# zhouxinlzu/PebbleSDR

Hardware: AMD Instinct MI355X
Metric: IQ Msamples/s through full ProcessBlock chain (higher is better)
Workload: dtype f32; 1 GPU; configs[1]: 20 Msps int8-shape IQ (values k/128, resident in HBM as float2), 1 channel/GPU, mixer+decimate(D=64)+WFM mono demod + 8192-bin SignalSpectrum per 2048-sample frame; frames_per_buffer=2048, spectrum_bins=8192, parallelism=independent channel per GPU, no collectives

## Files before the change

pebblesdr_amd/csrc/cores.hip:

```cpp
#include <cmath>
#include <cstdarg>
#include <cstddef>
#include <hip/hip_ext.h>
#include "kernels_demod.h"
#include "kernels_fastfir.h"
#include "kernels_frontend.h"
#include <algorithm>
#include "kernels_fused_dec.h"
#include "kernels_bank_dec.h"
#include "kernels_spectrum.h"
#include "receiver.h"

namespace pg {

std::string &last_error()
{
    static thread_local std::string e;
    return e;
}
int fail(int code, const char *fmt, ...)
{
    char buf[512];
    va_list ap;
    va_start(ap, fmt);
// ... 699 lines not shown
            }
            bank_state_valid = false;
        }
    }
    const long long len0 = max_in / s0.stride;
    if (ns == 1) {
        if (int rc = buf0.alloc((int)C, last_hist, len0)) return rc;
    } else {
        if (halo0 > 256 * 32) return fail(PEBBLEGPU_E_UNSUPPORTED, "cascade look-back %lld too deep", halo0);
        if (wide) {
            if (!fused_front) { if (int rc = buf0.alloc((int)C, wide_taps - 1, len0)) return rc; }
            if (int rc = buf1.alloc((int)C, (int)halo0, len0 / wide_stride)) return rc;
            if (int rc = fin.alloc((int)C, last_hist, len0 / wide_stride / later)) return rc;
        } else {
            if (int rc = buf0.alloc((int)C, (int)halo0, len0)) return rc;
            if (int rc = fin.alloc((int)C, last_hist, len0 / later)) return rc;
        }
    }
    for (int i = 0; i < 2; i++) {
        PG_HIP(hipMalloc((void **)&d_hist_mixed[i], sizeof(float2) * kMaxTaps * C));
        PG_HIP(hipMemset(d_hist_mixed[i], 0, sizeof(float2) * kMaxTaps * C));
        if (C == 1) {
            PG_HIP(hipMalloc((void **)&d_xtail_w[i], sizeof(float2) * 2048));
            PG_HIP(hipMemset(d_xtail_w[i], 0, sizeof(float2) * 2048));
        }

    }
    return 0;
}
void DecimCore::release()
{
    delete fused_p;
    fused_p = nullptr;
    for (int i = 0; i < 2; i++) {
        if (d_xhist[i]) (void)hipFree(d_xhist[i]);
        d_xhist[i] = nullptr;
    }
    for (int i = 0; i < 2; i++) {
        if (d_y0stage2[i]) (void)hipFree(d_y0stage2[i]);
        d_y0stage2[i] = nullptr;
    }
    d_y0stage = nullptr;
    for (int i = 0; i < 2; i++) {
        if (d_bank_state[i]) (void)hipFree(d_bank_state[i]);
        d_bank_state[i] = nullptr;
    }
    for (int i = 0; i < 2; i++) {
        if (d_dyn[i]) (void)hipFree(d_dyn[i]);
        d_dyn[i] = nullptr;
    }
    buf0.release();
    buf1.release();
    fin.release();
    fin2.release();
    fin3.release();
    if (d_wide_taps) (void)hipFree(d_wide_taps);
    d_wide_taps = nullptr;
    for (int i = 0; i < 2; i++) {
        if (d_hist_mixed[i]) (void)hipFree(d_hist_mixed[i]);
        d_hist_mixed[i] = nullptr;
        if (d_xtail_w[i]) (void)hipFree(d_xtail_w[i]);
        d_xtail_w[i] = nullptr;
    }
    if (d_c0tab) (void)hipFree(d_c0tab);
    d_c0tab = nullptr;
    if (d_ph_scratch) (void)hipFree(d_ph_scratch);
// ... 78 lines not shown
                                                            RawSrc raw)
{
    const int i = blockIdx.x * 256 + threadIdx.x;
    const long long src = n - 2048 + i;
    const float2 v = raw.base ? raw_load(raw, src) : in[src];
    out[i] = cscale(v, window[i]);
}
int DecimCore::run_beside_spectrum(hipStream_t s, const float2 *d_in, long long in_pitch, bool shared_input, long long n, const OscBank &osc, const RawSrc *raw)
{
    const int R = 8;
    const long long j_first = (10 + first.stride - 1) / first.stride;
    const RawSrc rs = raw ? *raw : RawSrc{nullptr, 0, 0, 0.f, 0};
    launch(raw ? k_mix_hb11_bank<false, false, true> : k_mix_hb11_bank<false, false, false>, dim3(len0 / (4LL * R * 64) != 0 ? 2 : 1, 1), dim3(256), s, d_in, in_pitch,
           (int)shared_input, buf0.data(), buf0.pitch, len0, (const ChanOsc *)osc.d_osc, (const float2 *)d_hist_mixed[hist_parity], d_hist_mixed[hist_parity ^ 1],
           (int)kMaxTaps, (const float *)osc.d_amp, osc.a_inf, bank_taps, first.gain, osc.inline_dyn, 0, (int)C, R, j_first, rs);
    PG_HIP(hipGetLastError());
    hist_parity ^= 1;
    xtail_parity ^= 1;
    last_fused = false;
    front_name = "k_spectrum_t128 (decimator inside)";
    rest_name = "";
    return 0;
}
int DecimCore::run(hipStream_t s, const float2 *d_in, long long in_pitch, bool shared_input, long long n, const OscBank &osc,
                   hipEvent_t after_first, const RawSrc *raw, const OscAdvance *oa)
{
    if (raw && !raw_ready(osc)) return fail(PEBBLEGPU_E_INVALID, "raw-format input reached a decimator path that has no converting loads");
    if (n <= 0 || n % (long long)chain.total != 0)
        return fail(PEBBLEGPU_E_SIZE, "%lld samples is not a multiple of the decimation %u", n, chain.total);
    len0 = n / first.stride;
    if (fin3.base && rotate3) { std::swap(fin, fin2); std::swap(fin2, fin3); }
    else if (fin2.base) std::swap(fin, fin2);
    const HistBuf *src = &buf0;
    last_fused = false;
    last_mfma = false;
    osc_advanced = false;
    done_recorded = false;
    const bool had_bank_state = bank_state_valid;
    bank_state_valid = false;
    const bool had_dyn = dyn_valid;
    dyn_valid = false;
    if ((fused_all || bank_mfma) && shared_input && !osc.any_transient()) {
        const HistBuf &y0b = fused_front ? buf1 : buf0;
        if (n / ((long long)first.stride * (fused_front ? wide_stride : 1)) > y0b.cap) return fail(PEBBLEGPU_E_SIZE, "%lld samples exceed this object's capacity", n);
        len_out = n / (long long)chain.total;
        const long long groups = cdiv(C, 64);
        if (bank_mfma && (unsigned long long)n * 8 < 0xFFF00000ull && (unsigned long long)C * (unsigned long long)fin.pitch * 8 < 0xFFF00000ull &&
            len_out >= 64 && (reinterpret_cast<uintptr_t>(d_in) & 7) == 0) {
            dyn_valid = had_dyn;
            if (int rc = run_bank_mfma(s, d_in, n, osc, had_bank_state, oa)) return rc;
            if (after_first) PG_HIP(hipEventRecord(after_first, s));
            return 0;
        }
      if (int rc = flush_y0(s)) return rc;
      if (fused_all) {
        long long L = tun.fused_l > 0 ? tun.fused_l : ((len_out * groups / 704 + 15) & ~15LL);
        if (L < 32) L = 32;
        fused_p->n_out = len_out;
        fused_p->out_pitch = fin.pitch;
        fused_p->y0_pitch = buf0.pitch;
        fused_p->L = (int)L;
        fused_p->a_inf = osc.a_inf;
        launch(k_mix_dec_fused<15, 19, 31>, dim3(cdiv(len_out, L), (unsigned)groups), dim3(256), s, d_in, fin.data(), (const ChanOsc *)osc.d_osc, osc.inline_dyn,
               (const float2 *)d_xhist[hist_parity], d_xhist[hist_parity ^ 1], (const float2 *)buf0.data(), d_y0stage, d_hist_mixed[hist_parity ^ 1], *fused_p);
        PG_HIP(hipGetLastError());
        hist_parity ^= 1;
// ... 5 lines not shown
      }
    }
    if (int rc = flush_y0(s)) return rc;
    if (fused_front) {
        len1 = len0 / wide_stride;
        if (len1 > buf1.cap) return fail(PEBBLEGPU_E_SIZE, "%lld samples exceed this object's capacity", n);
        int cl_log2 = 0;
        while ((1u << cl_log2) < C && cl_log2 < 6) cl_log2++;
        const int R = cl_log2 == 6 ? 16 : 8;
        const dim3 grid(cdiv(len1 + 1, 4LL * R * (64 >> cl_log2)), cdiv(C, 1u << cl_log2));
        const bool uni = cl_log2 == 6 && shared_input;
        auto kern = osc.any_transient() ? (uni ? k_mix_cic_hb<true, true> : k_mix_cic_hb<true, false>) : (uni ? k_mix_cic_hb<false, true> : k_mix_cic_hb<false, false>);
        launch_lds(kern, grid, dim3(256), cl_log2 ? 4 * (size_t)front_tile_slots(cl_log2, R) * sizeof(float2) : 0, s, d_in, in_pitch, (int)shared_input, buf1.data(), buf1.pitch,
                   len1, (const ChanOsc *)osc.d_osc, (const float2 *)d_hist_mixed[hist_parity], d_hist_mixed[hist_parity ^ 1], (int)kMaxTaps,
                   (const float *)osc.d_amp, osc.a_inf, wide_fir, first.stride, 1.0f, osc.inline_dyn, cl_log2, (int)C, R);
        hist_parity ^= 1;
        front_name = "k_mix_cic_hb";
        if (after_first) PG_HIP(hipEventRecord(after_first, s));
        len_out = len1;
        src = &buf1;
    } else {
        if (len0 > buf0.cap) return fail(PEBBLEGPU_E_SIZE, "%lld samples exceed this object's capacity", n);
        if (bank_front && C == 1 && want_lds_free && !osc.any_transient()) {
            const int R = 8;
            const long long j_first = (10 + first.stride - 1) / first.stride;
            const RawSrc rs = raw ? *raw : RawSrc{nullptr, 0, 0, 0.f, 0};
            auto lean = !raw ? k_mix_hb11_lean<-1> : rs.fmt == 0 ? k_mix_hb11_lean<0> : rs.fmt == 1 ? k_mix_hb11_lean<1> : rs.fmt == 2 ? k_mix_hb11_lean<2>
                             : rs.fmt == 3 ? k_mix_hb11_lean<3> : k_mix_hb11_lean<4>;
            const bool edge_launch = tun.lean_edge_launch;
            launch(lean, dim3(cdiv(len0, 4LL * R * 64) + (edge_launch ? 0 : 1)), dim3(256), s, d_in, buf0.data(), len0, (const ChanOsc *)osc.d_osc,
                   osc.a_inf, bank_taps, first.gain, osc.inline_dyn, R, edge_launch ? -j_first : j_first, rs, (const float2 *)d_hist_mixed[hist_parity],
                   d_hist_mixed[hist_parity ^ 1]);
            front_name = "k_mix_hb11_lean";
            if (edge_launch)
                launch(raw ? k_mix_hb11_bank<false, false, true> : k_mix_hb11_bank<false, false, false>, dim3(len0 / (4LL * R * 64) != 0 ? 2 : 1, 1), dim3(256), s, d_in, in_pitch,
                       (int)shared_input, buf0.data(), buf0.pitch, len0, (const ChanOsc *)osc.d_osc, (const float2 *)d_hist_mixed[hist_parity], d_hist_mixed[hist_parity ^ 1],
                       (int)kMaxTaps, (const float *)osc.d_amp, osc.a_inf, bank_taps, first.gain, osc.inline_dyn, 0, (int)C, R, j_first, rs);
        } else if (bank_front && (C >= 16 ? shared_input : want_lds_free)) {
            int cl_log2 = 0;
            while ((1u << cl_log2) < C && cl_log2 < 6) cl_log2++;
            const int R = cl_log2 == 6 ? 16 : 8;
            const dim3 grid(cdiv(len0 + 1, 4LL * R * (64 >> cl_log2)), cdiv(C, 1u << cl_log2));
            const bool uni = cl_log2 == 6;
            auto kern = osc.any_transient() ? (uni ? k_mix_hb11_bank<true, true> : k_mix_hb11_bank<true, false>)
                                            : (uni ? k_mix_hb11_bank<false, true> : k_mix_hb11_bank<false, false>);
            launch_lds(kern, grid, dim3(256), cl_log2 ? 4 * (size_t)front_tile_slots(cl_log2, R) * sizeof(float2) : 0, s, d_in, in_pitch, (int)shared_input, buf0.data(),
                       buf0.pitch, len0, (const ChanOsc *)osc.d_osc, (const float2 *)d_hist_mixed[hist_parity], d_hist_mixed[hist_parity ^ 1], (int)kMaxTaps,
                       (const float *)osc.d_amp, osc.a_inf, bank_taps, first.gain, osc.inline_dyn, cl_log2, (int)C, R, -1LL, RawSrc{nullptr, 0, 0, 0.f, 0});
            front_name = "k_mix_hb11_bank";
        } else {
        const int cg = (first.cic3 && first.stride > 2 && shared_input) ? 8 : 1;
        size_t lds = mixdec_lds_bytes(first);
        if (cg > 1 && lds < (size_t)cg * 258 * sizeof(float4)) lds = (size_t)cg * 258 * sizeof(float4);
        launch_lds(k_mix_dec1, dim3(cdiv(len0, 256), cdiv(C, cg)), dim3(256), lds, s, d_in, in_pitch, (int)shared_input, buf0.data(),
                   buf0.pitch, len0, (const ChanOsc *)osc.d_osc, (const float2 *)d_hist_mixed[hist_parity], (int)kMaxTaps, (const float *)osc.d_amp,
                   osc.a_inf, first, d_hist_mixed[hist_parity ^ 1], osc.inline_dyn, cg, (int)C);
        front_name = "k_mix_dec1";
        }
        hist_parity ^= 1;
        if (after_first) PG_HIP(hipEventRecord(after_first, s));
        len_out = len0;
        if (wide) {
            len1 = len0 / wide_stride;
            launch(k_fir_dec, dim3(cdiv(len1, 256), C), dim3(256), s, (const float2 *)buf0.data(), buf0.pitch, buf1.data(), buf1.pitch, len1, wide_stride,
                   (const float *)d_wide_taps, (const float *)nullptr, 0, (const int *)nullptr, wide_taps, 1.0f, 0, (const int *)nullptr, Gate{nullptr, 0, 0});
            src = &buf1;
        }
    }
    rest_name = wide && !fused_front ? "k_fir_dec" : "";
    if (casc.nst > 0) {
        rest_name = wide && !fused_front ? "k_fir_dec + k_cascade" : "k_cascade";
        len_out = n / (long long)chain.total;
        const bool three2 = casc.nst == 3 && casc.stride[0] == 2 && casc.stride[1] == 2 && casc.stride[2] == 2;
        auto kern = k_cascade<0, 0, 0>;
        if (three2 && casc.ntaps[0] == 15 && casc.ntaps[1] == 23 && casc.ntaps[2] == 47) kern = k_cascade<15, 23, 47>;
        else if (three2 && casc.ntaps[0] == 15 && casc.ntaps[1] == 19 && casc.ntaps[2] == 31) kern = k_cascade<15, 19, 31>;
        launch_lds(kern, dim3(cdiv(len_out, casc.outb), C), dim3(256), casc_lds_bytes, s, (const float2 *)src->data(), src->pitch, fin.data(),
                   fin.pitch, len_out, casc);
    }
    PG_HIP(hipGetLastError());
    if ((fused_all || bank_mfma) && shared_input && n >= xh_depth)
        PG_HIP(hipMemcpyAsync(d_xhist[hist_parity], d_in + (n - xh_depth), sizeof(float2) * xh_depth, hipMemcpyDeviceToDevice, s));
    if (fuse_window && n >= 2048 && shape_for_spectrum()) {
        launch(k_window_tail, dim3(8), dim3(256), s, d_in, n, fuse_window, d_xtail_w[xtail_parity ^ 1], raw ? *raw : RawSrc{nullptr, 0, 0, 0.f, 0});
        xtail_parity ^= 1;
    }
    return 0;
}
void DecimCore::tail_jobs_dec(std::vector<TailJob> &jobs) const
{
    if (last_fused) {
        const HistBuf &y0b = fused_front ? buf1 : buf0;
        if (!last_mfma) jobs.push_back(TailJob{d_y0stage, (long long)fused_hy, (long long)fused_hy, fused_hy, 0, y0b.base + (y0b.hist - fused_hy), y0b.pitch});
        return;
    }
    if (!fused_front && buf0.hist > 0 && casc.nst > 0) jobs.push_back(TailJob{buf0.data(), buf0.pitch, len0, buf0.hist, 0, nullptr, 0});
    if (wide && buf1.hist > 0) jobs.push_back(TailJob{buf1.data(), buf1.pitch, len1, buf1.hist, 0, nullptr, 0});
}
void DecimCore::tail_job_out(std::vector<TailJob> &jobs) const
{
    if (casc.nst == 0) {
        if (!fused_front && buf0.hist > 0) jobs.push_back(TailJob{buf0.data(), buf0.pitch, len0, buf0.hist, 0, nullptr, 0});
        return;
    }
    if (fin.hist <= 0) return;
    if (fin2.base) jobs.push_back(TailJob{fin.data(), fin.pitch, len_out, fin.hist, 0, fin2.base, fin2.pitch});
    else jobs.push_back(TailJob{fin.data(), fin.pitch, len_out, fin.hist, 0, nullptr, 0});
}
void DecimCore::tail_jobs(std::vector<TailJob> &jobs) const
// ... 315 lines not shown
        if (lp_on) ok = design::cascade_impulse(std::vector<double>(), nullptr, std::vector<design::Biquad>(1, l), 1e-11, kWfmLpMax, hl);
        if (ok) ok = design::cascade_impulse(h, &da, std::vector<design::Biquad>(1, br), 1e-11, kWfmIrMax, ha);
        fused = ok && wfm_fir_lds_bytes((int)((ha.size() + 15) & ~(size_t)15), (int)hl.size()) <= 64 * 1024;
        if (fused) {
            L4 = (int)((ha.size() + 15) & ~(size_t)15);
            Llp = (int)hl.size();
            ha.resize((size_t)L4 + 16, 0.0);
            std::vector<float> hlf(hl.begin(), hl.end()), haf(ha.begin(), ha.end());
            PG_HIP(hipMalloc((void **)&d_h, sizeof(float) * (L4 + 16)));
            PG_HIP(hipMemcpy(d_h, haf.data(), sizeof(float) * (L4 + 16), hipMemcpyHostToDevice));
            PG_HIP(hipMalloc((void **)&d_hlp, sizeof(float) * Llp));
            PG_HIP(hipMemcpy(d_hlp, hlf.data(), sizeof(float) * Llp, hipMemcpyHostToDevice));
            for (int i = 0; i < 2; i++) {
                PG_HIP(hipMalloc((void **)&d_xtail[i], sizeof(float2) * (size_t)(L4 + Llp) * C));
                PG_HIP(hipMemset(d_xtail[i], 0, sizeof(float2) * (size_t)(L4 + Llp) * C));
            }
            return 0;
        }
    }
    if (int rc = a.alloc((int)C, 2, max_n)) return rc;
    if (int rc = b.alloc((int)C, kMaxTaps, max_n)) return rc;
    if (int rc = c.alloc((int)C, 0, max_n)) return rc;
    for (int i = 0; i < 2; i++) {
        PG_HIP(hipMalloc((void **)&d_lp_state[i], sizeof(double) * 4 * C));
        PG_HIP(hipMemset(d_lp_state[i], 0, sizeof(double) * 4 * C));
        PG_HIP(hipMalloc((void **)&d_dn_state[i], sizeof(double) * 8 * C));
        PG_HIP(hipMemset(d_dn_state[i], 0, sizeof(double) * 8 * C));
    }
    return 0;
}
void WfmCore::release()
{
    a.release(); b.release(); c.release();
    void *p[] = {d_taps, d_lp_state[0], d_lp_state[1], d_dn_state[0], d_dn_state[1], d_h, d_hlp, d_xtail[0], d_xtail[1], d_stereo, d_pilot, d_hilb, d_stereo_list};
    d_stereo = nullptr;
    d_pilot = nullptr;
    d_hilb = nullptr;
    d_stereo_list = nullptr;
    lm.release();
    rds.release();
    for (void *q : p) if (q) (void)hipFree(q);
    d_taps = nullptr;
    d_lp_state[0] = d_lp_state[1] = d_dn_state[0] = d_dn_state[1] = nullptr;
    d_h = nullptr; d_hlp = nullptr; d_xtail[0] = d_xtail[1] = nullptr;
}
int WfmCore::set_stereo(uint32_t ch, bool on)
{
    if (ch >= C) return fail(PEBBLEGPU_E_INVALID, "channel %u out of range", ch);
    if (on && !fused) return fail(PEBBLEGPU_E_UNSUPPORTED, "dmFMS needs the single-kernel WFM path (this demodulator rate runs the sequential one)");
    if (on && !d_pilot) {
        const design::WfmPilotDesign pd = design::wfm_pilot_design(rate);
        memset(&pilot, 0, sizeof(pilot));
        pilot.b0 = pd.bp.b0; pilot.b2 = pd.bp.b2; pilot.a1 = pd.bp.a1; pilot.a2 = pd.bp.a2;
        pilot.nco_lo = pd.nco_lo; pilot.nco_hi = pd.nco_hi; pilot.alpha = pd.alpha; pilot.beta = pd.beta;
        pilot.err_alpha = pd.err_alpha; pilot.phase_adjust = pd.phase_adjust;
        pilot.L4 = L4;
        PG_HIP(hipMalloc((void **)&d_hilb, sizeof(double) * 122));
        PG_HIP(hipMemcpy(d_hilb, pd.hilb, sizeof(double) * 122, hipMemcpyHostToDevice));
        PG_HIP(hipMalloc((void **)&d_pilot, sizeof(WfmPilotState) * C));
        PG_HIP(hipMalloc((void **)&d_stereo_list, sizeof(int) * C));
        if (int rc = lm.alloc((int)C, L4 + 16, max_n_)) return rc;
        std::vector<WfmPilotState> z(C);
        memset(z.data(), 0, sizeof(WfmPilotState) * C);
        for (auto &q : z) { q.nco_freq = pd.nco_freq0; q.quiet = 1LL << 40; }
        PG_HIP(hipMemcpy(d_pilot, z.data(), sizeof(WfmPilotState) * C, hipMemcpyHostToDevice));
        if (tun.rds) { if (int rc = rds.init(C, rate, max_n_)) return rc; }
    }
// ... 20 lines not shown
int WfmCore::run(hipStream_t s, const float2 *in, long long in_pitch, float2 *out, long long out_pitch, long long n,
                 const std::vector<TailJob> *more_tails, const OscAdvance *oa, bool *carried)
{
    if (carried) *carried = false;
    if (n < kMaxTaps) return fail(PEBBLEGPU_E_SIZE, "WFM demod needs at least %d samples per call", kMaxTaps);
    last_n = n;
    if (stereo_dirty) {
        if (!d_stereo) PG_HIP(hipMalloc((void **)&d_stereo, C));
        PG_HIP(hipMemcpyAsync(d_stereo, stereo.data(), C, hipMemcpyHostToDevice, s));
        std::vector<int> list;
        for (uint32_t ch = 0; ch < C; ch++) if (stereo[ch]) list.push_back((int)ch);
        n_stereo = (int)list.size();
        if (n_stereo) PG_HIP(hipMemcpyAsync(d_stereo_list, list.data(), sizeof(int) * list.size(), hipMemcpyHostToDevice, s));
        PG_HIP(hipStreamSynchronize(s));
        stereo_dirty = false;
    }
    if (n_stereo) { if (int rc = rds.check(n, stereo_block)) return rc; }
    if (fused) {
        WfmFirParams wp;
        memset(&wp, 0, sizeof(wp));
        wp.L4 = L4;
        wp.Llp = Llp;
        wp.gain = 0.25f;
        const long long Lx = (long long)L4 + Llp;
        float2 *nt = d_xtail[parity ^ 1];
        deferred_in = nullptr;
        if (n >= Lx) {
            deferred_in = in;
            deferred_pitch = in_pitch;
        }
        const int groups = (int)cdiv(n, kWfmOutB);
        TailJobs tj;
        memset(&tj, 0, sizeof(tj));
        int extra = 0;
        if (more_tails != nullptr && n >= Lx) {
            std::vector<TailJob> jobs(*more_tails);
            jobs.push_back(TailJob{const_cast<float2 *>(in), in_pitch, n, (int)Lx, 0, nt, Lx});
            if (fill_tail_jobs(tj, jobs, oa) == 0) {
                extra = (int)jobs.size();
                if (carried) *carried = true;
                deferred_in = nullptr;
            } else {
                memset(&tj, 0, sizeof(tj));
            }
        }
        launch_lds(k_wfm_fir, dim3(groups + extra, C), dim3(512), wfm_fir_lds_bytes(L4, Llp), s, in, in_pitch, (const float2 *)d_xtail[parity],
                   out, out_pitch, n, wp, (const float *)d_h, (const float *)d_hlp, (const unsigned char *)d_stereo, groups, tj);
        PG_HIP(hipGetLastError());
        if (n < Lx) {
            PG_HIP(hipMemcpy2DAsync(nt, sizeof(float2) * Lx, d_xtail[parity] + n, sizeof(float2) * Lx, sizeof(float2) * (Lx - n), C, hipMemcpyDeviceToDevice, s));
            PG_HIP(hipMemcpy2DAsync(nt + (Lx - n), sizeof(float2) * Lx, in, sizeof(float2) * in_pitch, sizeof(float2) * n, C, hipMemcpyDeviceToDevice, s));
        }
        parity ^= 1;
        if (n_stereo) {
            if (last_lock.size() != C) { last_lock.assign(C, 1); stereo_ran.assign(C, 0); }
            for (uint32_t ch = 0; ch < C; ch++) if (stereo[ch]) stereo_ran[ch] = 1;
            if (n > lm.cap) return fail(PEBBLEGPU_E_SIZE, "%lld samples exceed this object's capacity", n);
            PG_HIP(hipMemset2DAsync(lm.data(), sizeof(float2) * (size_t)lm.pitch, 0, sizeof(float2) * (size_t)n, C, s));
            WfmPilotParams pp = pilot;
            pp.block = stereo_block > 0 ? stereo_block : (int)n;
            launch(k_wfm_pilot, dim3(cdiv(n_stereo, 64)), dim3(64), s, in, in_pitch, n, pp, (const double *)d_hilb, d_pilot, lm.data(), lm.pitch,
                   (const int *)d_stereo_list, n_stereo);
            launch(k_wfm_lmr_fir, dim3(cdiv(n, 256), n_stereo), dim3(256), s, (const float2 *)lm.data(), lm.pitch, (const float *)d_h, L4, out, out_pitch, n,
                   (const WfmPilotState *)d_pilot, (const int *)d_stereo_list);
            std::vector<TailJob> lj(1, TailJob{lm.data(), lm.pitch, n, lm.hist, 0, nullptr, 0});
            if (int rc = run_save_tails(s, lj, C)) return rc;
            PG_HIP(hipGetLastError());
            if (int rc = rds.run(s, in, in_pitch, n, (const double *)d_hilb, (const int *)d_stereo_list, n_stereo, stereo_block)) return rc;
        }
        return 0;
    }
    if (n > a.cap) return fail(PEBBLEGPU_E_SIZE, "%lld samples exceed this object's capacity", n);
    const long long nsub = (n + kSub - 1) / kSub;
    if (lp_on)
        launch(k_iir_scan<0, 1>, dim3(1, C), dim3(64), s, in, in_pitch, a.data(), a.pitch, n, lp, (const double *)d_lp_state[0], d_lp_state[0],
               (int)nsub, -1, (const int *)nullptr, Gate{nullptr, 0, 0});
    else
        launch(k_copy, dim3(cdiv(n, 256), C), dim3(256), s, in, in_pitch, a.data(), a.pitch, n);
// ... 730 lines not shown
```

pebblesdr_amd/csrc/kernels_demod.h:

```cpp
#pragma once
#include "params.h"
#include "tail_refresh.h"

namespace pg {


__device__ __forceinline__ int spad(int i) { return i + i / kSeg; }

__device__ __forceinline__ double sec_step(const ScanSection &S, double &s0, double &s1, double u)
{
    double y;
    if (S.type == kOnePoleDiff) {
        const double dn = (S.c[0] * s0) + u;
        y = dn - s0;
        s0 = dn;
    } else if (S.type == kOnePoleAvg) {
        s0 = (1.0 - S.c[0]) * s0 + S.c[0] * u;
        y = s0 * 2.0;
    } else {
        const double w0 = u - S.c[3] * s0 - S.c[4] * s1;
        y = S.c[0] * w0 + S.c[1] * s0 + S.c[2] * s1;
        s1 = s0;
        s0 = w0;
    }
// ... 193 lines not shown
        float ht[16];
#pragma unroll
        for (int u = 0; u < 4; u++) { ht[4 * u] = hn[u].x; ht[4 * u + 1] = hn[u].y; ht[4 * u + 2] = hn[u].z; ht[4 * u + 3] = hn[u].w; }
#pragma unroll
        for (int u = 0; u < 4; u++) hn[u] = hv[((p0 + 16) >> 2) + u];
        float a0 = 0.f, a1 = 0.f, a2 = 0.f, a3 = 0.f;
#pragma unroll
        for (int g = 0; g < 4; g++) {
            blk -= 1;
            const float4 prev = nxt;
            nxt = blk[-1];
            const float h0 = ht[4 * g], h1 = ht[4 * g + 1], h2 = ht[4 * g + 2], h3 = ht[4 * g + 3];
            a0 = fmaf(h0, cur.x, a0); a1 = fmaf(h0, cur.y, a1); a2 = fmaf(h0, cur.z, a2); a3 = fmaf(h0, cur.w, a3);
            a0 = fmaf(h1, prev.w, a0); a1 = fmaf(h1, cur.x, a1); a2 = fmaf(h1, cur.y, a2); a3 = fmaf(h1, cur.z, a3);
            a0 = fmaf(h2, prev.z, a0); a1 = fmaf(h2, prev.w, a1); a2 = fmaf(h2, cur.x, a2); a3 = fmaf(h2, cur.y, a3);
            a0 = fmaf(h3, prev.y, a0); a1 = fmaf(h3, prev.z, a1); a2 = fmaf(h3, prev.w, a2); a3 = fmaf(h3, cur.x, a3);
            cur = prev;
        }
        acc[0] += (double)a0; acc[1] += (double)a1; acc[2] += (double)a2; acc[3] += (double)a3;
    }
    __syncthreads();
    double *part = reinterpret_cast<double *>(xs);
    if (half) {
#pragma unroll
        for (int r = 0; r < 4; r++) part[r * 256 + ot] = acc[r];
    }
    __syncthreads();
    if (half) return;
    float2 *y = out + (long long)c * out_pitch + s + 4 * ot;
#pragma unroll
    for (int r = 0; r < 4; r++)
        if (s + 4 * ot + r < n) {
            const float v = (float)(acc[r] + part[r * 256 + ot]);
            y[r] = make_float2(v, v);
        }
}

static __global__ __launch_bounds__(64) void k_wfm_pilot(const float2 *__restrict__ in, long long in_pitch, long long n, WfmPilotParams pp,
                                                         const double *__restrict__ hilb, WfmPilotState *__restrict__ st,
                                                         float2 *__restrict__ lm, long long lm_pitch, const int *__restrict__ chan_list, int nlist)
{
    const int li = blockIdx.x * 64 + threadIdx.x;
    if (li >= nlist) return;
    const int c = chan_list[li];
    WfmPilotState *s = &st[c];
    const long long quiet0 = s->quiet;
    if (s->dropped) {
        s->skip = quiet0 >= (long long)pp.L4 ? 1 : 0;
        const long long q = quiet0 + n;
        s->quiet = q > (1LL << 40) ? (1LL << 40) : q;
        const float2 v = in[(long long)c * in_pitch + n - 1];
        s->d1_re = (double)v.x;
        s->d1_im = (double)v.y;
        return;
    }
    s->skip = 0;
    const double kTwoPi = 6.28318530717958647692528676656, kPiD = 3.14159265358979323846;
    const float2 *x = in + (long long)c * in_pitch;
    float2 *l = lm + (long long)c * lm_pitch;
    double d1r = s->d1_re, d1i = s->d1_im, w1a = s->w1a, w2a = s->w2a, w1b = s->w1b, w2b = s->w2b;
    double nco_phase = s->nco_phase, nco_freq = s->nco_freq, err_ave = s->err_ave;
    int zpos = s->zpos;
    long long quiet = quiet0;
    const double *hI = hilb, *hQ = hilb + 61;
    for (long long b0 = 0; b0 < n; b0 += pp.block) {
        const long long be = b0 + pp.block < n ? b0 + pp.block : n;
// ... 367 lines not shown
```

pebblesdr_amd/csrc/kernels_frontend.h:

```cpp
#pragma once
#include "params.h"
#include "tail_refresh.h"

namespace pg {


__device__ __forceinline__ float osc_amp(const float *__restrict__ amp_tab, float a_inf, uint32_t n0, long long i)
{
    unsigned long long k = (unsigned long long)n0 + (unsigned long long)i;
    return k < (unsigned long long)kAmpTab ? amp_tab[k] : a_inf;
}

static __global__ __launch_bounds__(256) void k_mixer(const float2 *__restrict__ in, long long in_pitch, int shared_input,
                                                float2 *__restrict__ out, long long out_pitch, long long n,
                                                const ChanOsc *__restrict__ osc, const float *__restrict__ amp_tab,
                                                float a_inf)
{
    const int c = blockIdx.y;
    const ChanOsc *o = &osc[c];
    const float2 *x = in + (shared_input ? 0 : (long long)c * in_pitch);
    float2 *y = out + (long long)c * out_pitch;
    const long long i0 = ((long long)blockIdx.x * 256 + threadIdx.x) * 4;
    if (i0 >= n) return;
    if (!o->mix_on) {
// ... 229 lines not shown
                            const float h = cp.h[s][p];
                            const float2 m = w[p];
                            acc.x = fmaf(m.x, h, acc.x);
                            acc.y = fmaf(m.y, h, acc.y);
                        }
                        if (last) out[(long long)c * out_pitch + o0 + j] = cscale(acc, cp.gain);
                        else dst[j] = acc;
                    }
                };
                if (s == 0) fixed(std::integral_constant<int, TF[0]>{});
                else if (s == 1) fixed(std::integral_constant<int, TF[1]>{});
                else fixed(std::integral_constant<int, TF[2]>{});
            } else
            for (int j = t; j < ns; j += 256) {
                const float2 *w = src + j * S;
                float2 acc = cscale(w[cc], ht[s][cc]);
                for (int p = 0; p < T; p += 2) {
                    const float h = ht[s][p];
                    const float2 m = w[p];
                    acc.x = fmaf(m.x, h, acc.x);
                    acc.y = fmaf(m.y, h, acc.y);
                }
                if (last) out[(long long)c * out_pitch + o0 + j] = cscale(acc, cp.gain);
                else dst[j] = acc;
            }
            __syncthreads();
            float2 *tmp = src;
            src = dst;
            dst = tmp;
        }
    }
}

__host__ __device__ inline int front_tile_slots(int cl_log2, int R) { return R * (64 >> cl_log2) * ((1 << cl_log2) + 1); }
__device__ __forceinline__ void front_store_rows(const float2 *__restrict__ tile, float2 *__restrict__ out, long long out_pitch, long long n_out,
                                                 int cbase, int n_chan, long long jb, int cl_log2, int R, int lane)
{
    const int CL = 1 << cl_log2, OL = 64 >> cl_log2;
    const int per_chan = R * OL;
    const int pl = __ffs(per_chan) - 1;
    wave_sync();
    for (int it = 0; it < R; it++) {
        const int idx = it * 64 + lane;
        const int ch = idx >> pl, jt = idx & (per_chan - 1);
        const long long j = jb + jt;
        if (cbase + ch < n_chan && j < n_out) out[(long long)(cbase + ch) * out_pitch + j] = tile[jt * (CL + 1) + ch];
    }
}

template <bool TRANSIENT, bool UNIFORM>
static __global__ __launch_bounds__(256) void k_mix_cic_hb(const float2 *__restrict__ in, long long in_pitch, int shared_input,
                                                            float2 *__restrict__ out, long long out_pitch, long long n_out,
                                                            const ChanOsc *__restrict__ osc, const float2 *__restrict__ hist,
                                                            float2 *__restrict__ hist_out, int hist_pitch, const float *__restrict__ amp_tab,
                                                            float a_inf, FrontTaps hb , int S0, float out_gain, OscDynInline dyn,
                                                            int cl_log2, int n_chan, int R)
{
    constexpr int T1 = kFrontT1, NP = T1 + 1;
    HIP_DYNAMIC_SHARED(float2, tiles)
    if (UNIFORM) cl_log2 = 6;
    const int lane = threadIdx.x & 63;
    const int wv = UNIFORM ? __builtin_amdgcn_readfirstlane(threadIdx.x >> 6) : (int)(threadIdx.x >> 6);
    const int CL = 1 << cl_log2, OL = 64 >> cl_log2;
    const int cl = lane & (CL - 1), ol = lane >> cl_log2;
    const int cbase = blockIdx.y * CL;
    const bool live = cbase + cl < n_chan;
// ... 435 lines not shown
```

pebblesdr_amd/csrc/receiver.h:

```cpp
#pragma once
#include <algorithm>
#include <complex>
#include <mutex>
#include <vector>
#include "../../include/pebblegpu.h"
#include "common.h"
#include "design.h"
#include "ingest.h"
#include "params.h"
#include "tuning.h"

namespace pg {

struct HistBuf {
    float2 *base = nullptr;
    long long pitch = 0;
    int hist = 0;
    long long cap = 0;
    int chans = 0;
    float2 *data(int c = 0) const { return base + (long long)c * pitch + hist; }
    int alloc(int channels, int hist_len, long long capacity);
    void release();
};

// ... 38 lines not shown
    float a_inf = 0;
    bool device_advance = false;
    bool dev_dyn_valid = false;
    double *d_adv = nullptr;
    uint64_t adv_n = 0;
    bool adv_stale = true;
    uint64_t dyn_epoch = 0;
    int advance_job(hipStream_t s, uint64_t n, OscAdvance *oa);
    int init(uint32_t channels, double sample_rate);
    void release();
    void retune(uint32_t ch, double f);
    void retune_keep(uint32_t ch, double f);
    bool force_mix = false;
    int upload(hipStream_t s);
    void advance(uint64_t n);
    bool any_transient() const;
};

bool bank_variant(int np, int t1, int t2, int t3, int *hy, int *nstate, int *minw);

struct DecimCore {
    design::Chain chain;
    uint32_t C = 0;
    FirTaps first;
    CascadeParams casc;
    size_t casc_lds_bytes = 0;
    HistBuf buf0, fin;
    bool wide = false;
    bool fused_front = false;
    FrontTaps wide_fir;
    bool bank_front = false;
    bool want_lds_free = false;
    bool front_is_lds_free() const { return C == 1 && (fused_front || bank_front); }
    FrontTaps bank_taps;
    bool fused_all = false, last_fused = false;
    struct FusedDecParams *fused_p = nullptr;
    float2 *d_xhist[2] = {nullptr, nullptr};
    float2 *d_y0stage = nullptr;
    float2 *d_y0stage2[2] = {nullptr, nullptr};
    int y0_cur = 0;
    int fused_hy = 0;
    bool bank_mfma = false;
    int bank_nstate = 0, bank_minw = 2;
    int run_bank_mfma(hipStream_t s, const float2 *d_in, long long n, const OscBank &osc, bool had_state, const OscAdvance *oa);
    int xh_depth = 16;
    float2 *d_bank_state[2] = {nullptr, nullptr};
    int bank_state_parity = 0;
    bool bank_state_valid = false;
    int wide_taps = 0, wide_stride = 1;
    float *d_wide_taps = nullptr;
    HistBuf buf1;
    long long len1 = 0;
    long long len0 = 0, len_out = 0;
    const char *front_name = "";
    const char *rest_name = "";
    float2 *d_hist_mixed[2] = {nullptr, nullptr};
    float2 *d_xtail_w[2] = {nullptr, nullptr};
    int xtail_parity = 0;
    const float *fuse_window = nullptr;
    float2 *d_c0tab = nullptr;
    std::vector<float> h_r0;
    std::vector<float2> h_c0;
    bool c0_valid = false;
    double c0_inc = 0;
    int c0_mix = 0;
    float2 *d_ph_scratch = nullptr;
// ... 172 lines not shown
    ScanParams<1> lp;
    ScanParams<2> dn;
    int warm_lp = -1, warm_dn = -1, parity = 0;
    double *d_lp_state[2] = {nullptr, nullptr}, *d_dn_state[2] = {nullptr, nullptr};
    bool fused = false;
    int L4 = 0, Llp = 1;
    float *d_h = nullptr;
    float *d_hlp = nullptr;
    float2 *d_xtail[2] = {nullptr, nullptr};
    const float2 *deferred_in = nullptr;
    long long deferred_pitch = 0;
    std::vector<unsigned char> stereo;
    unsigned char *d_stereo = nullptr;
    bool stereo_dirty = false;
    int set_stereo(uint32_t ch, bool on);
    HistBuf lm;
    struct WfmPilotState *d_pilot = nullptr;
    double *d_hilb = nullptr;
    int *d_stereo_list = nullptr;
    int n_stereo = 0;
    long long max_n_ = 0;
    int stereo_block = 2048;
    WfmPilotParams pilot;
    RdsCore rds;
    std::vector<char> stereo_ran, last_lock;
    int stereo_lock(hipStream_t s, uint32_t ch, int *lock, int *changed);
    Tuning tun;
    int init(uint32_t channels, double demod_rate, long long max_n, const Tuning &t);
    void release();
    int run(hipStream_t s, const float2 *in, long long in_pitch, float2 *out, long long out_pitch, long long n,
            const std::vector<TailJob> *more_tails = nullptr, const OscAdvance *oa = nullptr, bool *carried = nullptr);
    void tail_jobs(std::vector<TailJob> &jobs) const;
    long long last_n = 0;
};

struct AgcCore {
    uint32_t C = 0;
    double rate = 0;
    struct AgcState *d_state = nullptr;
    int *d_list = nullptr;
    std::vector<int> list;
    struct Host { int mode = 0, threshold = 1, use_hang = 0, thr = 0, decay = 0; double slope = 0, sample_rate = 100.0, manual = 1.0; bool dirty = false; };
    std::vector<Host> host;
    int init(uint32_t channels, double demod_rate);
    void release();
    int set_mode(uint32_t ch, int mode, int threshold);
    std::vector<char> muted;
    void set_muted(uint32_t ch, bool m) { if (muted.size() != C) muted.assign(C, 0); if ((muted[ch] != 0) != m) { muted[ch] = m; list_dirty = true; } }
    int apply(hipStream_t s);
    int run(hipStream_t s, float2 *buf, long long pitch, long long n, Gate gate = Gate{nullptr, 0, 0});
    bool list_dirty = false;
};

struct ConditionCore {
    uint32_t S = 0, nf = 0;
    double fs = 0;
    long long cap = 0;
    struct Host { int flags = 0; double gain = 1, phase = 0; };
    std::vector<Host> host;
    bool any = false, dirty = false;
    float2 *d_buf = nullptr;
    double *d_dc_state = nullptr;
    int *d_dc_list = nullptr;
    std::vector<int> dc_list;
    double2 *d_iq = nullptr;
    struct NbState *d_nb = nullptr;
// ... 209 lines not shown
```

pebblesdr_amd/csrc/receiver.hip:

```cpp
#include <cmath>
#include "receiver.h"

namespace pg {

static long long lcm_ll(long long a, long long b)
{
    long long x = a, y = b;
    while (y) { long long t = x % y; x = y; y = t; }
    return a / x * b;
}

int Receiver::create(const pebblegpu_config *cfg)
{
    device = cfg->device;
    fs = cfg->sample_rate;
    nf = cfg->frames_per_buffer ? cfg->frames_per_buffer : 2048;
    C = cfg->n_channels;
    shared_input = cfg->shared_input != 0;
    S = shared_input ? 1 : C;
    wfm = cfg->wfm != 0;
    bins = cfg->spectrum_bins;
    ff_n = cfg->fastfir_fft ? cfg->fastfir_fft : 2048;
    ff_taps = cfg->fastfir_taps ? cfg->fastfir_taps : 1025;
    max_sf = cfg->max_superframes ? cfg->max_superframes : 1;
// ... 515 lines not shown
    if (with_spectrum && gated()) {
        sel_spec_.clear();
        ut_spec_.advance(spec_ups_, spec_period_ms_, n / nf, nf, (uint64_t)fs, &sel_spec_);
        const long long ns = (long long)sel_spec_.size();
        if (int rc = measure_carry(stream_)) return rc;
        if (int rc = spec_.run_list(stream_, d_iq, in_pitch, sel_spec_.data(), ns, d_spec, raw)) return rc;
        last_spec_frames = (uint64_t)ns;
        if (ns) {
            if (smeter_on) { if (int rc = run_signal_strength(stream_, d_spec, ns * (long long)bins, (int)bins, ns, d_sm_bins, d_smeter, smeter_pitch, C)) return rc; }
            PG_HIP(hipMemcpy2DAsync(d_spec_carry, sizeof(float) * bins, d_spec + (ns - 1) * (long long)bins, sizeof(float) * (size_t)ns * bins, sizeof(float) * bins, S,
                                    hipMemcpyDeviceToDevice, stream_));
            have_carry_ = true;
        }
    } else if (with_spectrum) {
        ut_spec_.advance(-1, 0, n / nf, nf, (uint64_t)fs, nullptr);
        if (int rc = spec_.run(stream_, d_iq, in_pitch, (long long)(n / nf), d_spec, raw, fuse_dec ? &df : nullptr, !side)) return rc;
        last_spec_frames = n / nf;
        if (smeter_on) {
            const long long F = (long long)(n / nf);
            if (int rc = run_signal_strength(stream_, d_spec, F * (long long)bins, (int)bins, F, d_sm_bins, d_smeter, smeter_pitch, C)) return rc;
        }
    }
    const bool mid = with_spectrum || profile_detail || side;
    if (mid) PG_HIP(hipEventRecord(ev[1], stream_));
    tm.detailed[(tm.calls - 1) % Timers::kRing] = profile_detail;
    tm.has_mid[(tm.calls - 1) % Timers::kRing] = mid;
    if (!with_chain) {
        if (profile_detail) for (int i = 2; i <= 5; i++) PG_HIP(hipEventRecord(ev[i], stream_));
        PG_HIP(hipEventRecord(ev[6], stream_));
        guard.armed = false;
        return 0;
    }
    dec_.want_lds_free = side;
    OscAdvance oa_pre;
    memset(&oa_pre, 0, sizeof(oa_pre));
    bool have_oa = false;
    if (fuse_dec) {
        if (int rc = dec_.run_beside_spectrum(cs, d_iq, in_pitch, shared_input, (long long)n, osc_, raw)) return rc;
        PG_HIP(hipStreamWaitEvent(cs, ev[1], 0));
    } else {
        if (!wfm) {
            if (int rc = osc_.advance_job(cs, n, &oa_pre)) return rc;
            have_oa = true;
        }
        dec_.done_event = nullptr;
        if (bank_pipe && tun_.bank_pipe_extev) {
            if (!sync_ev_[0]) for (hipEvent_t &e : sync_ev_) PG_HIP(hipEventCreateWithFlags(&e, hipEventDisableTiming));
            dec_.done_event = sync_ev_[tm.calls % 4];
        }
        if (int rc = dec_.run(cs, d_iq, in_pitch, shared_input, (long long)n, osc_, profile_detail ? ev[2] : nullptr, raw, have_oa ? &oa_pre : nullptr)) return rc;
        dec_.done_event = nullptr;
        if (have_oa && dec_.osc_advanced) memset(&oa_pre, 0, sizeof(oa_pre));
    }
    if (profile_detail) PG_HIP(hipEventRecord(ev[3], cs));
    if (bank_pipe) {
        std::vector<TailJob> jobs;
        dec_.tail_jobs_dec(jobs);
        const bool nothing_behind = jobs.empty() && oa_pre.osc == nullptr;
        if (int rc = run_save_tails(stream_, jobs, C, &oa_pre)) return rc;
        const bool timed_ev = tun_.bank_pipe_timed_ev;
        if (!sync_ev_[0]) for (hipEvent_t &e : sync_ev_) PG_HIP(hipEventCreateWithFlags(&e, hipEventDisableTiming));
        pipe_ev_ = timed_ev ? ev[1] : sync_ev_[tm.calls % 4];
        if (!(dec_.done_recorded && nothing_behind && !timed_ev)) PG_HIP(hipEventRecord(pipe_ev_, stream_));
        cs = chain_stream_;
        PG_HIP(hipStreamWaitEvent(cs, pipe_ev_, 0));
        const int nap = tun_.bank_pipe_nap;
// ... 141 lines not shown
    osc_.advance(n);
    guard.armed = false;
    return 0;
}

int Receiver::process_raw(int fmt, int order, double gain, const void *d_raw, uint64_t n)
{
    if (!d_raw || n == 0) return fail(PEBBLEGPU_E_INVALID, "null input or zero samples");
    if (fmt < 0 || fmt > 4 || order < 0 || order > 3) return fail(PEBBLEGPU_E_INVALID, "unknown sample format %d / IQ order %d", fmt, order);
    if (n > (uint64_t)max_sf * superframe) return fail(PEBBLEGPU_E_SIZE, "%llu samples exceed this object's capacity", (unsigned long long)n);
    const RawSrc raw{d_raw, fmt, order, raw_scale(fmt, gain), 0};
    return process(nullptr, n, bins != 0, true, &raw);
}

int Receiver::ingest_acquire(uint32_t slot, uint64_t bytes, void **host_ptr) { return ingest_.acquire(device, slot, bytes, host_ptr); }
int Receiver::ingest_submit(uint32_t slot, uint64_t bytes) { return ingest_.submit(device, slot, bytes); }
int Receiver::process_ingested(uint32_t slot, int fmt, int order, double gain, uint64_t n)
{
    IngestSlot *g = nullptr;
    if (int rc = ingest_.check(slot, fmt, (uint64_t)S * n, n, &g)) return rc;
    PG_HIP(hipSetDevice(device));
    if (int rc = ingest_.wait_upload(*g, stream_, chain_stream_)) return rc;
    if (int rc = process_raw(fmt, order, gain, g->d, n)) return rc;
    return ingest_.mark_in_flight(*g, stream_, chain_stream_);
}

const char *Receiver::kernel_name(int which) const
{
    switch (which) {
    case 1: return !bins ? "" : gated() ? (spec_.any ? "k_spectrum_list_any" : "k_spectrum_list_q128") : spec_.big ? "k_big256_cols + k_big256_rows" : spec_.per_q ? "k_spectrum_q128" : bins == 8192 ? (spec_.use_w64 ? "k_spectrum_w64" : spec_.last_fullc ? "k_spectrum_t128 (twiddles held)" : "k_spectrum_t128") : bins == 4096 ? "k_spectrum<2>" : "k_spectrum_1to1";
    case 2: return dec_.front_name;
    case 3: return dec_.rest_name;
    case 4: return wfm ? "" : ff_n == 2048 ? "k_fastfir_t128" : "k_fastfir";
    case 5: return wfm ? (wfmc_.fused ? "k_wfm_fir" : "k_iir_scan + k_discrim + k_fir_dec") : "k_anf/k_agc/k_iir_scan/k_pll_demod + k_fir_dec (listed channels only)";
    default: return "";
    }
}

int Receiver::close_timing()
{
    if (tm.open_slot >= 0) {
        PG_HIP(hipEventRecord(tm.ev[tm.open_slot][6], stream_));
        tm.end_ev[tm.open_slot] = tm.ev[tm.open_slot][6];
        tm.open_slot = -1;
    }
    return 0;
}

int Receiver::map_spectrum(bool zoom, const int32_t *edges, bool per_stream, int32_t y_pixels, int32_t x_pixels, double max_db, double min_db,
                           uint32_t first, uint32_t n, uint32_t step, int32_t *d_out)
{
    std::lock_guard<std::mutex> g(mu_);
    if (!d_out || !edges) return fail(PEBBLEGPU_E_INVALID, "null argument");
    if (int rc = check_screen_map(y_pixels, x_pixels, max_db, min_db)) return rc;
    if (failed_) return fail(PEBBLEGPU_E_HIP, "an earlier call on this receiver failed half-way: its spectra are not defined");
    const uint32_t fft = zoom ? zoom_bins : bins;
    uint64_t frames = zoom ? last_zoom_frames : last_spec_frames;
    const bool carried = !zoom && gated() && !frames && have_carry_;
    if (carried) frames = 1;
    if (!fft) return fail(PEBBLEGPU_E_INVALID, zoom ? "the receiver computes no zoomed spectrum (hires_bins = 0)" : "the receiver computes no spectrum (spectrum_bins = 0)");
    if (!frames) return fail(PEBBLEGPU_E_INVALID, "no call with a spectrum has been made yet");
    if (n == 0 || (uint64_t)first + (uint64_t)(n - 1) * step >= frames)
        return fail(PEBBLEGPU_E_INVALID, "frames %u + j * %u, j < %u, are not all within the last call's %llu", first, step, n, (unsigned long long)frames);
    PG_HIP(hipSetDevice(device));
    if (int rc = close_timing()) return rc;
    const int rows = zoom ? (int)C : (int)S;
    const float *src = carried ? d_spec_carry : (zoom ? d_zoom : d_spec) + (long long)first * fft;
// ... 65 lines not shown
```

pebblesdr_amd/csrc/tail_refresh.h:

```cpp
#pragma once
#include "params.h"

namespace pg {

__device__ __forceinline__ void save_tails_block(const TailJobs &jobs, int z, int y, int tid)
{
    if (jobs.oa.osc != nullptr && z == 0 && tid == 0 && (uint32_t)y < jobs.oa.osc_count) {
        ChanOsc &o = jobs.oa.osc[y];
        double p = o.phase0 + jobs.oa.adv[y];
        p -= floor(p);
        o.phase0 = p >= 1.0 ? 0.0 : p;
        const uint32_t n0 = o.n0 + jobs.oa.adv_n;
        o.n0 = n0 > (uint32_t)kAmpTab ? (uint32_t)kAmpTab : n0;
    }
    if (z >= jobs.count) return;
    const TailJob &tj = jobs.job[z];
    float2 *b = tj.data + (long long)y * tj.pitch;
    float2 keep[32];
    if (tid < 256) {
#pragma unroll
        for (int k = 0; k < 32; k++) {
            const int j = tid + 256 * k;
            if (j < tj.hist) keep[k] = b[tj.n - tj.hist + j];
        }
    }
    __syncthreads();
    if (tid < 256) {
#pragma unroll
        for (int k = 0; k < 32; k++) {
            const int j = tid + 256 * k;
            if (j < tj.hist) {
                if (tj.dst) tj.dst[(long long)y * tj.dst_pitch + j] = keep[k];
                else b[-tj.hist + j] = keep[k];
            }
        }
    }
}

}
```

Before: 123,900 Msamples/s.

## Add LDS-free lean cascade and split WFM discriminator/audio kernels for single channel

For the single-channel WFM configuration, replaces the LDS-based cascade decimator with a kernel that stages intermediate results in a global scratch slab. It also splits the fused WFM FIR kernel into a discriminator kernel that writes a float buffer and an audio FIR kernel that reads it with float4 loads. The goal is to raise occupancy by dropping LDS and register pressure (launch_bounds 256,8; smaller tail-save arrays). The cost is extra global memory traffic, one more launch, and new scratch allocations.

After: 113,600 Msamples/s. 8.3% lower.

```diff
diff --git a/pebblesdr_amd/csrc/cores.hip b/pebblesdr_amd/csrc/cores.hip
--- a/pebblesdr_amd/csrc/cores.hip
+++ b/pebblesdr_amd/csrc/cores.hip
@@ -755,6 +755,9 @@
 {
     delete fused_p;
     fused_p = nullptr;
+    if (d_slab) (void)hipFree(d_slab);
+    d_slab = nullptr;
+    slab_cap = 0;
     for (int i = 0; i < 2; i++) {
         if (d_xhist[i]) (void)hipFree(d_xhist[i]);
         d_xhist[i] = nullptr;
@@ -899,6 +902,7 @@
     if (fin3.base && rotate3) { std::swap(fin, fin2); std::swap(fin2, fin3); }
     else if (fin2.base) std::swap(fin, fin2);
     const HistBuf *src = &buf0;
+    bool lean_front = false;
     last_fused = false;
     last_mfma = false;
     osc_advanced = false;
@@ -970,6 +974,7 @@
                    osc.a_inf, bank_taps, first.gain, osc.inline_dyn, R, edge_launch ? -j_first : j_first, rs, (const float2 *)d_hist_mixed[hist_parity],
                    d_hist_mixed[hist_parity ^ 1]);
             front_name = "k_mix_hb11_lean";
+            lean_front = true;
             if (edge_launch)
                 launch(raw ? k_mix_hb11_bank<false, false, true> : k_mix_hb11_bank<false, false, false>, dim3(len0 / (4LL * R * 64) != 0 ? 2 : 1, 1), dim3(256), s, d_in, in_pitch,
                        (int)shared_input, buf0.data(), buf0.pitch, len0, (const ChanOsc *)osc.d_osc, (const float2 *)d_hist_mixed[hist_parity], d_hist_mixed[hist_parity ^ 1],
@@ -1013,6 +1018,21 @@
         auto kern = k_cascade<0, 0, 0>;
         if (three2 && casc.ntaps[0] == 15 && casc.ntaps[1] == 23 && casc.ntaps[2] == 47) kern = k_cascade<15, 23, 47>;
         else if (three2 && casc.ntaps[0] == 15 && casc.ntaps[1] == 19 && casc.ntaps[2] == 31) kern = k_cascade<15, 19, 31>;
+        if (lean_front && want_lean_tail && lean_tail_shape()) {
+            const long long groups = cdiv(len_out, casc.outb);
+            const int a_slots = ((casc.outb * 2 + 46) * 2 + 22 + 15) & ~15, b_slots = (casc.outb * 2 + 46 + 15) & ~15;
+            const size_t need = (size_t)groups * (size_t)(a_slots + b_slots);
+            if (need > slab_cap) {
+                if (d_slab) (void)hipFree(d_slab);
+                d_slab = nullptr;
+                slab_cap = 0;
+                PG_HIP(hipMalloc((void **)&d_slab, sizeof(float2) * need));
+                slab_cap = need;
+            }
+            launch_lds(k_cascade_lean<15, 23, 47>, dim3((unsigned)groups), dim3(256), 0 , s, (const float2 *)src->data(),
+                       fin.data(), len_out, casc, d_slab, a_slots, a_slots + b_slots);
+            rest_name = "k_cascade_lean";
+        } else
         launch_lds(kern, dim3(cdiv(len_out, casc.outb), C), dim3(256), casc_lds_bytes, s, (const float2 *)src->data(), src->pitch, fin.data(),
                    fin.pitch, len_out, casc);
     }
@@ -1394,7 +1414,9 @@
 void WfmCore::release()
 {
     a.release(); b.release(); c.release();
-    void *p[] = {d_taps, d_lp_state[0], d_lp_state[1], d_dn_state[0], d_dn_state[1], d_h, d_hlp, d_xtail[0], d_xtail[1], d_stereo, d_pilot, d_hilb, d_stereo_list};
+    void *p[] = {d_taps, d_lp_state[0], d_lp_state[1], d_dn_state[0], d_dn_state[1], d_h, d_hlp, d_xtail[0], d_xtail[1], d_stereo, d_pilot, d_hilb, d_stereo_list, d_disc};
+    d_disc = nullptr;
+    disc_cap = 0;
     d_stereo = nullptr;
     d_pilot = nullptr;
     d_hilb = nullptr;
@@ -1481,7 +1503,7 @@
         const int groups = (int)cdiv(n, kWfmOutB);
         TailJobs tj;
         memset(&tj, 0, sizeof(tj));
-        int extra = 0;
+        int extra = 0, deepest = 0;
         if (more_tails != nullptr && n >= Lx) {
             std::vector<TailJob> jobs(*more_tails);
             jobs.push_back(TailJob{const_cast<float2 *>(in), in_pitch, n, (int)Lx, 0, nt, Lx});
@@ -1489,10 +1511,27 @@
                 extra = (int)jobs.size();
                 if (carried) *carried = true;
                 deferred_in = nullptr;
+                for (const TailJob &j : jobs) deepest = std::max(deepest, j.hist);
             } else {
                 memset(&tj, 0, sizeof(tj));
             }
         }
+        last_lean = want_lean && C == 1 && n_stereo == 0 && extra > 0 && deepest <= 256 * 4;
+        if (last_lean) {
+            const size_t front = (size_t)L4 + 16, need = front + (size_t)groups * kWfmOutB;
+            if (need > disc_cap) {
+                if (d_disc) (void)hipFree(d_disc);
+                d_disc = nullptr;
+                disc_cap = 0;
+                PG_HIP(hipMalloc((void **)&d_disc, sizeof(float) * need));
+                disc_cap = need;
+                PG_HIP(hipMemsetAsync(d_disc, 0, sizeof(float) * need, s));
+            }
+            float *d0 = d_disc + front;
+            launch_lds(k_wfm_disc_lean, dim3((unsigned)cdiv(n + L4, 256)), dim3(256), 0, s, in, (const float2 *)d_xtail[parity], d0, n, wp, (const float *)d_hlp);
+            launch_lds(k_wfm_audio_lean, dim3(groups + extra), dim3(256), 0 , s, (const float *)d0, out, n, wp,
+                       (const float *)d_h, groups, tj);
+        } else
         launch_lds(k_wfm_fir, dim3(groups + extra, C), dim3(512), wfm_fir_lds_bytes(L4, Llp), s, in, in_pitch, (const float2 *)d_xtail[parity],
                    out, out_pitch, n, wp, (const float *)d_h, (const float *)d_hlp, (const unsigned char *)d_stereo, groups, tj);
         PG_HIP(hipGetLastError());
diff --git a/pebblesdr_amd/csrc/kernels_demod.h b/pebblesdr_amd/csrc/kernels_demod.h
--- a/pebblesdr_amd/csrc/kernels_demod.h
+++ b/pebblesdr_amd/csrc/kernels_demod.h
@@ -249,6 +249,88 @@
     for (int r = 0; r < 4; r++)
         if (s + 4 * ot + r < n) {
             const float v = (float)(acc[r] + part[r * 256 + ot]);
+            y[r] = make_float2(v, v);
+        }
+}
+
+static __global__ __launch_bounds__(256, 8) void k_wfm_disc_lean(const float2 *__restrict__ in, const float2 *__restrict__ xtail, float *__restrict__ d,
+                                                                  long long n, WfmFirParams wp, const float *__restrict__ hlp)
+{
+    const int L4 = wp.L4, Llp = wp.Llp, Lx = L4 + Llp;
+    const long long t = (long long)blockIdx.x * 256 + threadIdx.x - L4;
+    if (t >= n) return;
+    const float2 *xt = xtail + Lx;
+    float2 c0 = make_float2(0.f, 0.f), c1 = make_float2(0.f, 0.f);
+    auto taps = [&](auto sample) {
+        float2 v = sample(t);
+        float hp = hlp[0];
+        c0.x = fmaf(hp, v.x, c0.x);
+        c0.y = fmaf(hp, v.y, c0.y);
+#pragma unroll 8
+        for (int m = 1; m < Llp; m++) {
+            v = sample(t - m);
+            const float h = hlp[m];
+            c0.x = fmaf(h, v.x, c0.x);
+            c0.y = fmaf(h, v.y, c0.y);
+            c1.x = fmaf(hp, v.x, c1.x);
+            c1.y = fmaf(hp, v.y, c1.y);
+            hp = h;
+        }
+        v = sample(t - Llp);
+        c1.x = fmaf(hp, v.x, c1.x);
+        c1.y = fmaf(hp, v.y, c1.y);
+    };
+    if ((long long)blockIdx.x * 256 - Lx < 0) taps([&](long long g) { return g < 0 ? xt[g] : in[g]; });
+    else taps([&](long long g) { return in[g]; });
+    d[t] = wp.gain * atan2f(c1.x * c0.y - c0.x * c1.y, c1.x * c0.x + c1.y * c0.y);
+}
+
+static __global__ __launch_bounds__(256, 8) void k_wfm_audio_lean(const float *__restrict__ d, float2 *__restrict__ out, long long n, WfmFirParams wp,
+                                                                   const float *__restrict__ h, int n_fir_groups, TailJobs tails)
+{
+    if ((int)blockIdx.x >= n_fir_groups) {
+        save_tails_block<4>(tails, (int)blockIdx.x - n_fir_groups, 0, (int)threadIdx.x);
+        return;
+    }
+    const int L4 = wp.L4, ot = threadIdx.x;
+    const long long s = (long long)blockIdx.x * kWfmOutB;
+    const int p_split = ((L4 >> 1) + 15) & ~15;
+    double acc[2][4] = {{0.0, 0.0, 0.0, 0.0}, {0.0, 0.0, 0.0, 0.0}};
+    const float4 *base = reinterpret_cast<const float4 *>(d + s) + ot;
+#pragma unroll
+    for (int half = 0; half < 2; half++) {
+        const int p_lo = half ? p_split : 0, p_hi = half ? L4 : p_split;
+        const float4 *blk = base - (p_lo >> 2);
+        float4 cur = blk[0];
+        float4 nb[4];
+#pragma unroll
+        for (int g = 0; g < 4; g++) nb[g] = blk[-1 - g];
+        for (int p0 = p_lo; p0 < p_hi; p0 += 16) {
+            float4 b[4];
+#pragma unroll
+            for (int g = 0; g < 4; g++) b[g] = nb[g];
+            blk -= 4;
+#pragma unroll
+            for (int g = 0; g < 4; g++) nb[g] = blk[-1 - g];
+            float a0 = 0.f, a1 = 0.f, a2 = 0.f, a3 = 0.f;
+#pragma unroll
+            for (int g = 0; g < 4; g++) {
+                const float4 prev = b[g];
+                const float h0 = h[p0 + 4 * g], h1 = h[p0 + 4 * g + 1], h2 = h[p0 + 4 * g + 2], h3 = h[p0 + 4 * g + 3];
+                a0 = fmaf(h0, cur.x, a0); a1 = fmaf(h0, cur.y, a1); a2 = fmaf(h0, cur.z, a2); a3 = fmaf(h0, cur.w, a3);
+                a0 = fmaf(h1, prev.w, a0); a1 = fmaf(h1, cur.x, a1); a2 = fmaf(h1, cur.y, a2); a3 = fmaf(h1, cur.z, a3);
+                a0 = fmaf(h2, prev.z, a0); a1 = fmaf(h2, prev.w, a1); a2 = fmaf(h2, cur.x, a2); a3 = fmaf(h2, cur.y, a3);
+                a0 = fmaf(h3, prev.y, a0); a1 = fmaf(h3, prev.z, a1); a2 = fmaf(h3, prev.w, a2); a3 = fmaf(h3, cur.x, a3);
+                cur = prev;
+            }
+            acc[half][0] += (double)a0; acc[half][1] += (double)a1; acc[half][2] += (double)a2; acc[half][3] += (double)a3;
+        }
+    }
+    float2 *y = out + s + 4 * ot;
+#pragma unroll
+    for (int r = 0; r < 4; r++)
+        if (s + 4 * ot + r < n) {
+            const float v = (float)(acc[0][r] + acc[1][r]);
             y[r] = make_float2(v, v);
         }
 }
diff --git a/pebblesdr_amd/csrc/kernels_frontend.h b/pebblesdr_amd/csrc/kernels_frontend.h
--- a/pebblesdr_amd/csrc/kernels_frontend.h
+++ b/pebblesdr_amd/csrc/kernels_frontend.h
@@ -285,6 +285,39 @@
     }
 }
 
+template <int F0, int F1, int F2>
+static __global__ __launch_bounds__(256, 8) void k_cascade_lean(const float2 *__restrict__ in, float2 *__restrict__ out, long long n_out, CascadeParams cp,
+                                                                 float2 *slab, int slab_b, int slab_stride)
+{
+    const int t = threadIdx.x;
+    const long long o0 = (long long)blockIdx.x * cp.outb;
+    const int nfin = (int)((n_out - o0) < cp.outb ? (n_out - o0) : cp.outb);
+    const int n2 = nfin * 2 + F2 - 1, n1 = n2 * 2 + F1 - 1;
+    const long long first = ((o0 * 2 - (F2 - 1)) * 2 - (F1 - 1)) * 2 - (F0 - 1);
+    float2 *ya = slab + (long long)blockIdx.x * slab_stride, *yb = ya + slab_b;
+    auto stage = [&](auto tc, int s, const float2 *src, float2 *dst, int ns, bool last) {
+        constexpr int TT = decltype(tc)::value, CC = (TT - 1) >> 1;
+        for (int j = t; j < ns; j += 256) {
+            const float2 *w = src + j * 2;
+            float2 acc = cscale(w[CC], cp.h[s][CC]);
+#pragma unroll
+            for (int p = 0; p < TT; p += 2) {
+                const float h = cp.h[s][p];
+                const float2 m = w[p];
+                acc.x = fmaf(m.x, h, acc.x);
+                acc.y = fmaf(m.y, h, acc.y);
+            }
+            if (last) out[o0 + j] = cscale(acc, cp.gain);
+            else dst[j] = acc;
+        }
+    };
+    stage(std::integral_constant<int, F0>{}, 0, in + first, ya, n1, false);
+    __syncthreads();
+    stage(std::integral_constant<int, F1>{}, 1, ya, yb, n2, false);
+    __syncthreads();
+    stage(std::integral_constant<int, F2>{}, 2, yb, nullptr, nfin, true);
+}
+
 __host__ __device__ inline int front_tile_slots(int cl_log2, int R) { return R * (64 >> cl_log2) * ((1 << cl_log2) + 1); }
 __device__ __forceinline__ void front_store_rows(const float2 *__restrict__ tile, float2 *__restrict__ out, long long out_pitch, long long n_out,
                                                  int cbase, int n_chan, long long jb, int cl_log2, int R, int lane)
diff --git a/pebblesdr_amd/csrc/receiver.h b/pebblesdr_amd/csrc/receiver.h
--- a/pebblesdr_amd/csrc/receiver.h
+++ b/pebblesdr_amd/csrc/receiver.h
@@ -94,6 +94,11 @@
     bool bank_front = false;
     bool want_lds_free = false;
     bool front_is_lds_free() const { return C == 1 && (fused_front || bank_front); }
+    bool want_lean_tail = false;
+    bool lean_tail_shape() const { return C == 1 && !wide && casc.nst == 3 && casc.stride[0] == 2 && casc.stride[1] == 2 && casc.stride[2] == 2 &&
+                                          casc.ntaps[0] == 15 && casc.ntaps[1] == 23 && casc.ntaps[2] == 47; }
+    float2 *d_slab = nullptr;
+    size_t slab_cap = 0;
     FrontTaps bank_taps;
     bool fused_all = false, last_fused = false;
     struct FusedDecParams *fused_p = nullptr;
@@ -332,6 +337,9 @@
             const std::vector<TailJob> *more_tails = nullptr, const OscAdvance *oa = nullptr, bool *carried = nullptr);
     void tail_jobs(std::vector<TailJob> &jobs) const;
     long long last_n = 0;
+    bool want_lean = false, last_lean = false;
+    float *d_disc = nullptr;
+    size_t disc_cap = 0;
 };
 
 struct AgcCore {
diff --git a/pebblesdr_amd/csrc/receiver.hip b/pebblesdr_amd/csrc/receiver.hip
--- a/pebblesdr_amd/csrc/receiver.hip
+++ b/pebblesdr_amd/csrc/receiver.hip
@@ -571,6 +571,9 @@
         return 0;
     }
     dec_.want_lds_free = side;
+    const bool lean_tail = side && wfm && !fuse_dec && !gated() && S == 1 && bins == 8192 && !spec_.big && !spec_.per_q && !spec_.any && !spec_.use_w64;
+    dec_.want_lean_tail = lean_tail;
+    wfmc_.want_lean = lean_tail;
     OscAdvance oa_pre;
     memset(&oa_pre, 0, sizeof(oa_pre));
     bool have_oa = false;
@@ -778,7 +781,7 @@
     case 2: return dec_.front_name;
     case 3: return dec_.rest_name;
     case 4: return wfm ? "" : ff_n == 2048 ? "k_fastfir_t128" : "k_fastfir";
-    case 5: return wfm ? (wfmc_.fused ? "k_wfm_fir" : "k_iir_scan + k_discrim + k_fir_dec") : "k_anf/k_agc/k_iir_scan/k_pll_demod + k_fir_dec (listed channels only)";
+    case 5: return wfm ? (wfmc_.fused ? (wfmc_.last_lean ? "k_wfm_disc_lean + k_wfm_audio_lean" : "k_wfm_fir") : "k_iir_scan + k_discrim + k_fir_dec") : "k_anf/k_agc/k_iir_scan/k_pll_demod + k_fir_dec (listed channels only)";
     default: return "";
     }
 }
diff --git a/pebblesdr_amd/csrc/tail_refresh.h b/pebblesdr_amd/csrc/tail_refresh.h
--- a/pebblesdr_amd/csrc/tail_refresh.h
+++ b/pebblesdr_amd/csrc/tail_refresh.h
@@ -3,6 +3,7 @@
 
 namespace pg {
 
+template <int K = 32>
 __device__ __forceinline__ void save_tails_block(const TailJobs &jobs, int z, int y, int tid)
 {
     if (jobs.oa.osc != nullptr && z == 0 && tid == 0 && (uint32_t)y < jobs.oa.osc_count) {
@@ -16,10 +17,10 @@
     if (z >= jobs.count) return;
     const TailJob &tj = jobs.job[z];
     float2 *b = tj.data + (long long)y * tj.pitch;
-    float2 keep[32];
+    float2 keep[K];
     if (tid < 256) {
 #pragma unroll
-        for (int k = 0; k < 32; k++) {
+        for (int k = 0; k < K; k++) {
             const int j = tid + 256 * k;
             if (j < tj.hist) keep[k] = b[tj.n - tj.hist + j];
         }
@@ -27,7 +28,7 @@
     __syncthreads();
     if (tid < 256) {
 #pragma unroll
-        for (int k = 0; k < 32; k++) {
+        for (int k = 0; k < K; k++) {
             const int j = tid + 256 * k;
             if (j < tj.hist) {
                 if (tj.dst) tj.dst[(long long)y * tj.dst_pitch + j] = keep[k];
```
